# atomicarchitects/equiformer

Hardware: AMD Instinct MI355X
Metric: molecules/sec (train step) QM9 L_max=2, 6 blocks (higher is better)
Workload: dtype f32; 1 GPU; QM9 graph_attention_transformer_nonlinear_l2 train step (radius graph + fwd + L1 + bwd + AdamW), 128 molecules/GPU x 18 atoms, r=5.0, num_basis=128, alpha_drop=0.2; global_batch=128, nodes_per_gpu=2304, edges_per_gpu=25354, parallelism=dp1, matrix_mode=split, hip_graph=True, hip_graph_replays=455, hip_graph_eager_steps=3

## Files before the change

### equiformer_amd/csrc/common.h

```cpp
#pragma once
#include <hip/hip_runtime.h>
#include <stdint.h>
#include "../../include/equiformer_hip.h"

#define EQF_CHECK_LAUNCH()                      \
  do {                                          \
    hipError_t e__ = hipGetLastError();         \
    if (e__ != hipSuccess) return (int)e__;     \
  } while (0)

static inline int eqf_cdiv(long a, long b) { return (int)((a + b - 1) / b); }

__device__ __forceinline__ float wave_sum(float v) {
#pragma unroll
  for (int o = 32; o > 0; o >>= 1) v += __shfl_xor(v, o);
  return v;
}
__device__ __forceinline__ float wave_max(float v) {
#pragma unroll
  for (int o = 32; o > 0; o >>= 1) v = fmaxf(v, __shfl_xor(v, o));
  return v;
}
__device__ __forceinline__ float half_sum(float v) {
#pragma unroll
  for (int o = 16; o > 0; o >>= 1) v += __shfl_xor(v, o);
  return v;
}

__device__ __forceinline__ float sigmoidf_(float x) { return 1.0f / (1.0f + __expf(-x)); }

__device__ __forceinline__ long row_off2(int i, int d, int ld, int inner) {
  if (d == 1) return (long)i * ld;
  int q;
  if (i < (1 << 21)) q = (int)(((float)i + 0.5f) * __builtin_amdgcn_rcpf((float)d));
  else q = i / d;
  int r = i - q * d;
  return (long)q * ld + (long)r * inner;
}

struct SmallDiv {
  int d;
  float inv;
  __device__ __forceinline__ explicit SmallDiv(int d_) : d(d_), inv(1.0f / (float)d_) {}
  __device__ __forceinline__ int div(int t) const { return (int)(((float)t + 0.5f) * inv); }
};

__host__ __device__ inline int irreps_dim(const eqf_irreps& ir) {
  int D = 0;
  for (int s = 0; s < ir.nseg; ++s) D += ir.mul[s] * (2 * ir.l[s] + 1);
  return D;
}
```

### equiformer_amd/csrc/gemmx.hip

```cpp
#include <climits>
#include "sfcx_common.h"

namespace {

constexpr int GX_BK = 32;
constexpr int GX_LDK = 40;
constexpr int GX_T = 64;
constexpr int GX_ROW = GX_T * GX_LDK;
constexpr int GX_MAXP = 24;

typedef __bf16 bf16x4_t __attribute__((ext_vector_type(4)));

struct GRows {
  const float* base;
  int d, ld, inner;
};

struct GXP {
  GRows A, B, C;
  const float* bias;
  float* cs;
  float* Cw;
  int ldc;
  int M, N, K;
  int accumulate, kind;
  int vecA, vecB;
  int steps_per_split;
};
static_assert(sizeof(GXP) * GX_MAXP + 4 * (2 * GX_MAXP + 3) <= 4000, "kernarg segment");
struct GXGroup {
  int n;
  int woff[GX_MAXP + 1];
  GXP p[GX_MAXP];
};

__device__ __forceinline__ int flat_problem(const GXGroup& g, int b) {
  int pi = 0;
#pragma unroll
  for (int j = 1; j < GX_MAXP; ++j) pi += (int)((unsigned)(g.woff[j] - 1 - b) >> 31);
  return pi;
}

template <int NP>
__device__ __forceinline__ void split_n(const float* v, int n, __bf16 (*p)[8]) {
#pragma unroll
  for (int j = 0; j < 8; ++j) {
    if (j >= n) break;
    float r = v[j];
#pragma unroll
    for (int q = 0; q < NP; ++q) {
      const __bf16 h = (__bf16)r;
      p[q][j] = h;
      if (q + 1 < NP) r = r - (float)h;
    }
  }
}

template <int NP>
struct LoaderKC {
  float4 v[2];
  long roff[2];
  bool rv[2];
  __device__ __forceinline__ void init(const GRows& R, int x0, int X) {
    const int xr0 = threadIdx.x >> 3;
#pragma unroll
    for (int pass = 0; pass < 2; ++pass) {
      const int x = x0 + xr0 + 32 * pass;
      rv[pass] = x < X;
      roff[pass] = row_off2(rv[pass] ? x : x0, R.d, R.ld, R.inner);
    }
  }
  int krem;
  template <bool VEC>
  __device__ __forceinline__ void issue(const GRows& R, int k0, int K) {
    const int k = k0 + 4 * (threadIdx.x & 7);
    krem = K - k;
    if constexpr (VEC) {
      const int kc = krem > 0 ? k : 0;
#pragma unroll
      for (int pass = 0; pass < 2; ++pass) v[pass] = *reinterpret_cast<const float4*>(R.base + roff[pass] + kc);
    } else {
#pragma unroll
      for (int pass = 0; pass < 2; ++pass) {
        const float* const p = R.base + roff[pass];
        v[pass] = make_float4(p[min(k, K - 1)], p[min(k + 1, K - 1)], p[min(k + 2, K - 1)], p[min(k + 3, K - 1)]);
      }
    }
  }
  __device__ __forceinline__ void commit(__bf16* __restrict__ T) const {
    const int kq = threadIdx.x & 7, xr0 = threadIdx.x >> 3;
#pragma unroll
    for (int pass = 0; pass < 2; ++pass) {
      float f[4] = {v[pass].x, v[pass].y, v[pass].z, v[pass].w};
#pragma unroll
      for (int e = 0; e < 4; ++e)
        if (!(rv[pass] && e < krem)) f[e] = 0.f;
      __bf16 p[NP][8];
      split_n<NP>(f, 4, p);
#pragma unroll
      for (int q = 0; q < NP; ++q)
        *reinterpret_cast<bf16x4_t*>(T + q * GX_ROW + (xr0 + 32 * pass) * GX_LDK + 4 * kq) =
            bf16x4_t{p[q][0], p[q][1], p[q][2], p[q][3]};
    }
  }
};

template <int NP>
struct LoaderKS {
  float v[8];
// ... 70 lines not shown
  for (int half = 0; half < 2; ++half) {
    __builtin_amdgcn_fence(__ATOMIC_ACQ_REL, "wavefront");
    __builtin_amdgcn_wave_barrier();
#pragma unroll
    for (int q8 = 0; q8 < 8; ++q8) T[((q8 & 3) + 8 * (q8 >> 2) + 4 * hi) * GX_ST_LD + r] = acc[8 * half + q8];
    __builtin_amdgcn_fence(__ATOMIC_ACQ_REL, "wavefront");
    __builtin_amdgcn_wave_barrier();
#pragma unroll
    for (int k = 0; k < 2; ++k) {
      const int lr = rr + 8 * k, grow = row0 + 16 * half + lr;
      f32x4 v = *reinterpret_cast<const f32x4*>(T + lr * GX_ST_LD + c4);
      if (grow < M && col0 + c4 < N) {
        float* const p = rowptr(grow) + (col0 + c4);
        if (accumulate) {
          const f32x4 o = *reinterpret_cast<const f32x4*>(p);
          v[0] += o[0], v[1] += o[1], v[2] += o[2], v[3] += o[3];
        }
        *reinterpret_cast<f32x4*>(p) = v;
      }
    }
  }
}

template <int MODE, int BKIND, bool VEC>
__global__ __launch_bounds__(256) void gemmx_rows_kernel(const GXGroup g_byval) {
  KERNARG_IN_PLACE(GXGroup);
  constexpr int NA = Planes<MODE>::A, NB = Planes<MODE>::W;
  const int pi = flat_problem(g, (int)blockIdx.x);
  const GXP& P = g.p[pi];
  const int local = (int)blockIdx.x - g.woff[pi], tiles_n = (P.N + GX_T - 1) / GX_T;
  const int mt = local / tiles_n;
  const int m0 = mt * GX_T, n0 = (local - mt * tiles_n) * GX_T;
  __shared__ __attribute__((aligned(16))) __bf16 As[2][NA * GX_ROW];
  __shared__ __attribute__((aligned(16))) __bf16 Bs[2][NB * GX_ROW];
  const int wave = threadIdx.x >> 6;
  const int wm0 = (wave >> 1) * 32, wn0 = (wave & 1) * 32;
  f32x16 acc;
#pragma unroll
  for (int q = 0; q < 16; ++q) acc[q] = 0.f;

  LoaderKC<NA> la;
  LoaderKC<NB> lbk;
  LoaderKS<NB> lbs;
  la.init(P.A, m0, P.M);
  la.template issue<VEC>(P.A, 0, P.K);
  if constexpr (BKIND == 1) {
    lbk.init(P.B, n0, P.N);
    lbk.template issue<VEC>(P.B, 0, P.K);
  } else {
    lbs.init(P.B, 0);
    lbs.issue(P.B, P.K, n0, P.N);
  }
  la.commit(As[0]);
  if constexpr (BKIND == 1) lbk.commit(Bs[0]);
  else lbs.commit(Bs[0], false);
  __syncthreads();
  int cur = 0;
  for (int k0 = 0; k0 < P.K; k0 += GX_BK) {
    const bool more = k0 + GX_BK < P.K;
    if (more) {
      la.template issue<VEC>(P.A, k0 + GX_BK, P.K);
      if constexpr (BKIND == 1) lbk.template issue<VEC>(P.B, k0 + GX_BK, P.K);
      else lbs.issue(P.B, P.K, n0, P.N);
    }
    gx_mma<NA, NB>(As[cur], Bs[cur], wm0, wn0, acc);
    if (more) {
      la.commit(As[cur ^ 1]);
      if constexpr (BKIND == 1) lbk.commit(Bs[cur ^ 1]);
      else lbs.commit(Bs[cur ^ 1], false);
    }
    __syncthreads();
    cur ^= 1;
  }

  const int lane = threadIdx.x & 63, r = lane & 31, hi = lane >> 5;
  const int col = n0 + wn0 + r;
  const float bv = (P.bias && col < P.N) ? P.bias[col] : 0.f;
  const bool flat_c = P.C.d == 1;
  const SmallDiv cdiv(P.C.d);
  float* const cbase = const_cast<float*>(P.C.base);
  const int rb = m0 + wm0 + 4 * hi;
  static_assert(sizeof(As) >= 4 * GX_ST_FLOATS * sizeof(float), "the operand stages double as the store tiles");
  if (((P.C.ld | P.C.inner | P.N) & 3) == 0 && (reinterpret_cast<size_t>(cbase) & 15) == 0) {
#pragma unroll
    for (int q = 0; q < 16; ++q) acc[q] += bv;
    gx_store_tile16(acc, reinterpret_cast<float*>(&As[0][0]) + wave * GX_ST_FLOATS, m0 + wm0, P.M, n0 + wn0, P.N, P.accumulate != 0,
                    lane, [&](const int grow) {
                      if (flat_c) return cbase + (long)grow * P.C.ld;
                      const int qd = grow / P.C.d;
// ... 29 lines not shown
    }
  }
}

constexpr int GW_K = 64;
constexpr int GW_LDK = GW_K + 8;
constexpr int GW_ROW = GX_T * GW_LDK;

template <int NP>
struct LoaderWide {
  float4 v[GW_K / 16];
  int kv;
  __device__ __forceinline__ void issue(const GRows& R, int x0, int X, int K, bool two_level) {
    const int row = x0 + (threadIdx.x >> 2), q = threadIdx.x & 3;
    const bool rv = row < X;
    kv = rv ? K : 0;
    const long off = two_level ? row_off2(rv ? row : x0, R.d, R.ld, R.inner) : (long)(rv ? row : x0) * R.ld;
#pragma unroll
    for (int j = 0; j < GW_K / 16; ++j) {
      const int k = 4 * (q + 4 * j);
      v[j] = *reinterpret_cast<const float4*>(R.base + off + (k < K ? k : 0));
    }
  }
  __device__ __forceinline__ void commit(__bf16* __restrict__ T) const {
    const int row = threadIdx.x >> 2, q = threadIdx.x & 3;
#pragma unroll
    for (int j = 0; j < GW_K / 16; ++j) {
      const bool ok = 4 * (q + 4 * j) < kv;
      const float f[4] = {ok ? v[j].x : 0.f, ok ? v[j].y : 0.f, ok ? v[j].z : 0.f, ok ? v[j].w : 0.f};
      __bf16 p[NP][8];
      split_n<NP>(f, 4, p);
#pragma unroll
      for (int pl = 0; pl < NP; ++pl)
        *reinterpret_cast<bf16x4_t*>(T + pl * GW_ROW + row * GW_LDK + 4 * (q + 4 * j)) = bf16x4_t{p[pl][0], p[pl][1], p[pl][2], p[pl][3]};
    }
  }
};

template <int MODE>
__global__ __launch_bounds__(256) void gemmx_rows_wide_kernel(const GXGroup g_byval) {
  KERNARG_IN_PLACE(GXGroup);
  constexpr int NA = Planes<MODE>::A, NB = Planes<MODE>::W;
  const GXP& P = g.p[blockIdx.z];
  const int m0 = blockIdx.x * GX_T;
  if (m0 >= P.M) return;
  __shared__ __attribute__((aligned(16))) __bf16 As[NA * GW_ROW];
  __shared__ __attribute__((aligned(16))) __bf16 Bs[NB * GW_ROW];
  __shared__ __attribute__((aligned(16))) float St[4 * GX_ST_FLOATS];
  const int wave = threadIdx.x >> 6, lane = threadIdx.x & 63, r = lane & 31, hi = lane >> 5;
  const int wm0 = (wave >> 1) * 32, wn0 = (wave & 1) * 32;
  LoaderWide<NA> la;
  LoaderWide<NB> lb;
  la.issue(P.A, m0, P.M, P.K, true);
  lb.issue(P.B, 0, P.N, P.K, false);
  la.commit(As);
  const bool flat_c = P.C.d == 1;
  const SmallDiv cdiv(P.C.d);
  float* const cbase = const_cast<float*>(P.C.base);
  const int rb = m0 + wm0 + 4 * hi;
  long off0;
  int rem0 = 0;
  if (flat_c) {
    off0 = (long)rb * P.C.ld;
  } else {
    const int qb = rb / P.C.d;
    rem0 = rb - qb * P.C.d;
    off0 = (long)qb * P.C.ld;
  }
  const int nkt = (P.K + 15) / 16;
  const bool vec_c = ((P.C.ld | P.C.inner | P.N) & 3) == 0 && (reinterpret_cast<size_t>(cbase) & 15) == 0;
  for (int n0 = 0; n0 < P.N; n0 += GX_T) {
    __syncthreads();
    lb.commit(Bs);
    __syncthreads();
    if (n0 + GX_T < P.N) lb.issue(P.B, n0 + GX_T, P.N, P.K, false);
    f32x16 acc;
#pragma unroll
// ... 89 lines not shown
    __syncthreads();
    cur ^= 1;
  }
  {
    const int x = threadIdx.x & 63;
    if (csA && m0 + x < P.M) atomicAdd(P.cs + m0 + x, la.cs);
    if (csB && n0 + x < P.N) atomicAdd(P.cs + n0 + x, lb.cs);
  }
  const int lane = threadIdx.x & 63, r = lane & 31, hi = lane >> 5;
  const int col = n0 + wn0 + r;
  if (col >= P.N) return;
#pragma unroll
  for (int q = 0; q < 16; ++q) {
    const int row = m0 + wm0 + (q & 3) + 8 * (q >> 2) + 4 * hi;
    if (row < P.M) atomicAdd(P.Cw + (long)row * P.ldc + col, acc[q]);
  }
}

inline bool aligned16(const void* p) { return (reinterpret_cast<uintptr_t>(p) & 15) == 0; }
inline bool rows_vec_ok(const float* base, const eqf_rows& r) { return aligned16(base) && (r.ld % 4 == 0) && (r.inner % 4 == 0); }

static int g_gemmx_tn_minsteps = 8;

}

extern "C" {

int eqf_gemmx_group(const eqf_gemm_desc* d, int n, int mode, void* stream) {
  if (!d || n < 1 || n > GX_MAXP || mode < 0 || mode > 2) return EQF_E_BADARG;
  hipStream_t st = (hipStream_t)stream;
  for (int i = 0; i < n; ++i) {
    if (d[i].kind < 0 || d[i].kind > 3) return EQF_E_BADARG;
    if (!d[i].A || !d[i].B || !d[i].C || d[i].ra.d < 1 || d[i].rc.d < 1) return EQF_E_BADARG;
    if (d[i].kind < 2 && d[i].K < 1) return EQF_E_BADARG;
  }
  static thread_local GXGroup G;
  for (int kind = 0; kind < 2; ++kind) {
    memset(&G, 0, sizeof G);
    int maxm = 0, big = 0, wide_ok = 1, vec_ok = 1, wg = 0;
    double flops = 0, bytes = 0;
    for (int i = 0; i < n; ++i) {
      if (d[i].kind != kind || d[i].M <= 0 || d[i].N <= 0) continue;
      GXP& P = G.p[G.n];
      G.woff[G.n++] = wg;
      wg += eqf_cdiv(d[i].M, GX_T) * eqf_cdiv(d[i].N, GX_T);
      P.A = {d[i].A, d[i].ra.d, d[i].ra.ld, d[i].ra.inner};
      P.B = {d[i].B, 1, d[i].ldb, 0};
      P.C = {d[i].C, d[i].rc.d, d[i].rc.ld, d[i].rc.inner};
      P.bias = d[i].bias;
      P.M = d[i].M, P.N = d[i].N, P.K = d[i].K, P.accumulate = d[i].accumulate, P.kind = kind;
      P.vecA = rows_vec_ok(d[i].A, d[i].ra);
      P.vecB = aligned16(d[i].B) && d[i].ldb % 4 == 0;
      if (P.K % 4 != 0 || !P.vecA || (kind == 1 && !P.vecB)) vec_ok = 0;
      if (!(kind == 1 && P.K <= GW_K && P.K % 4 == 0 && P.vecA && P.vecB && P.M >= 8192 && P.N >= 2 * GX_T)) wide_ok = 0;
      if (eqf_cdiv(P.M, GX_T) > maxm) maxm = eqf_cdiv(P.M, GX_T);
      if (P.M >= 32768 / 2 + 1) big = 1;
      flops += 2.0 * P.M * (double)P.N * P.K;
      bytes += 4.0 * ((double)P.M * P.K + (double)P.K * P.N + (double)P.M * P.N);
    }
    if (G.n == 0) continue;
    const bool wide = kind == 1 && wide_ok;
    for (int i = G.n; i <= GX_MAXP; ++i) G.woff[i] = i == G.n ? wg : INT_MAX;
    const dim3 grid = wide ? dim3(maxm, 1, G.n) : dim3(wg, 1, 1);
    const int pid = eqf_prof_begin(kind == 0 ? (big ? "gemmx_group_kn_edge" : "gemmx_group_kn_node")
                                             : (big ? "gemmx_group_nk_edge" : "gemmx_group_nk_node"), st, flops, bytes);
#define GX_ROWS(M_)                                                                                              \
  do {                                                                                                           \
    if (wide) {                                                                                                  \
      hipLaunchKernelGGL((gemmx_rows_wide_kernel<M_>), grid, dim3(256), 0, st, G);                              \
    } else if (kind == 0) {                                                                                      \
      if (vec_ok) hipLaunchKernelGGL((gemmx_rows_kernel<M_, 0, true>), grid, dim3(256), 0, st, G);              \
      else hipLaunchKernelGGL((gemmx_rows_kernel<M_, 0, false>), grid, dim3(256), 0, st, G);                    \
    } else {                                                                                                     \
      if (vec_ok) hipLaunchKernelGGL((gemmx_rows_kernel<M_, 1, true>), grid, dim3(256), 0, st, G);              \
      else hipLaunchKernelGGL((gemmx_rows_kernel<M_, 1, false>), grid, dim3(256), 0, st, G);                    \
    }                                                                                                            \
  } while (0)
    if (mode == 0) GX_ROWS(0);
    else if (mode == 1) GX_ROWS(1);
    else GX_ROWS(2);
#undef GX_ROWS
    eqf_prof_end(pid, st);
    EQF_CHECK_LAUNCH();
  }
  {
    memset(&G, 0, sizeof G);
    int big = 0, wg = 0;
    double flops = 0, bytes = 0;
    for (int i = 0; i < n; ++i) {
      if (d[i].kind != 2 && d[i].kind != 3) continue;
      if (d[i].M <= 0 || d[i].N <= 0 || d[i].K <= 0) continue;
// ... 12 lines not shown
      ksplit = eqf_cdiv(total_steps, P.steps_per_split);
      G.woff[G.n] = wg;
      wg += tiles * ksplit;
      G.n++;
      if (P.K >= 32768 / 2 + 1) big = 1;
      flops += 2.0 * P.M * (double)P.N * P.K;
      bytes += 4.0 * ((double)P.K * P.M + (double)P.K * P.N + (double)P.M * P.N);
    }
    if (G.n > 0) {
      for (int i = G.n; i <= GX_MAXP; ++i) G.woff[i] = i == G.n ? wg : INT_MAX;
      const dim3 grid(wg, 1, 1);
      const int pid = eqf_prof_begin(big ? "gemmx_group_tn_edge" : "gemmx_group_tn_node", st, flops, bytes);
      if (mode == 0) hipLaunchKernelGGL((gemmx_tn_kernel<0>), grid, dim3(256), 0, st, G);
      else if (mode == 1) hipLaunchKernelGGL((gemmx_tn_kernel<1>), grid, dim3(256), 0, st, G);
      else hipLaunchKernelGGL((gemmx_tn_kernel<2>), grid, dim3(256), 0, st, G);
      eqf_prof_end(pid, st);
      EQF_CHECK_LAUNCH();
    }
  }
  return 0;
}

}
```

### equiformer_amd/csrc/rowops.hip

```cpp
#include "common.h"

namespace {

constexpr int WAVES_PER_BLOCK = 4;

struct SegTab {
  int nseg;
  int off[EQF_MAX_SEG];
  int len[EQF_MAX_SEG];
  int mul[EQF_MAX_SEG];
  int l[EQF_MAX_SEG];
  int woff[EQF_MAX_SEG];
  int boff[EQF_MAX_SEG];
  int zidx[EQF_MAX_SEG];
  int n0;
  int D;
};

SegTab make_segtab(const eqf_irreps& ir) {
  SegTab t{};
  t.nseg = ir.nseg;
  int off = 0, w = 0, b = 0, n0 = 0;
  for (int s = 0; s < ir.nseg; ++s) {
    t.off[s] = off;
// ... 307 lines not shown
    o.x = c * g.x * dsilu(v.x), o.y = c * g.y * dsilu(v.y), o.z = c * g.z * dsilu(v.z), o.w = c * g.w * dsilu(v.w);
    reinterpret_cast<float4*>(dx)[i] = o;
  }
  if (i == 0)
    for (long j = n4 * 4; j < n; ++j) dx[j] = c * dy[j] * dsilu(x[j]);
}

__global__ __launch_bounds__(256) void lnsilu_fwd_kernel(const float* __restrict__ x, const float* __restrict__ gamma,
                                                         const float* __restrict__ beta, float* __restrict__ y, int rows,
                                                         int C, float eps, int G) {
  const long ld = (long)G * C;
  {
    const int g_ = blockIdx.y * C;
    x += g_;
    gamma += g_;
    beta += g_;
    y += g_;
  }
  const int lane = threadIdx.x & 63;
  const int row = blockIdx.x * WAVES_PER_BLOCK + (threadIdx.x >> 6);
  if (row >= rows) return;
  const bool act = lane < C;
  const float v = act ? x[(long)row * ld + lane] : 0.f;
  const float mean = wave_sum(v) / C;
  const float d = act ? v - mean : 0.f;
  const float rs = rsqrtf(wave_sum(d * d) / C + eps);
  if (act) {
    const float z = d * rs * gamma[lane] + beta[lane];
    y[(long)row * ld + lane] = z * sigmoidf_(z);
  }
}

__global__ __launch_bounds__(256) void lnsilu_bwd_kernel(const float* __restrict__ x, const float* __restrict__ gamma,
                                                         const float* __restrict__ beta, const float* __restrict__ dy,
                                                         float* __restrict__ dx, float* __restrict__ d_gamma,
                                                         float* __restrict__ d_beta, int rows, int C, float eps, int G) {
  const long ld = (long)G * C;
  {
    const int g_ = blockIdx.y * C;
    x += g_;
    gamma += g_;
    beta += g_;
    dy += g_;
    dx += g_;
    d_gamma += g_;
    d_beta += g_;
  }
  const int lane = threadIdx.x & 63;
  const int wave_global = blockIdx.x * WAVES_PER_BLOCK + (threadIdx.x >> 6);
  const int nwaves = gridDim.x * WAVES_PER_BLOCK;
  const bool act = lane < C;
  const float gm = act ? gamma[lane] : 0.f, bt = act ? beta[lane] : 0.f;
  float acc_g = 0.f, acc_b = 0.f;
// ... 410 lines not shown
```

### equiformer_amd/lib.py

```python
import ctypes
import os

_HERE = os.path.dirname(os.path.abspath(__file__))
LIB_PATH = os.path.join(_HERE, "libequiformer_hip.so")
if os.environ.get("EQF_LIB_VARIANT"):
    LIB_PATH = os.path.join(_HERE, "libequiformer_hip_%s.so" % os.environ["EQF_LIB_VARIANT"])

EQF_MAX_SEG = 8
EQF_MAX_PATHS = 72

c_fp = ctypes.c_void_p
c_int = ctypes.c_int


class EqfIrreps(ctypes.Structure):
    _fields_ = [("nseg", c_int), ("l", c_int * EQF_MAX_SEG), ("mul", c_int * EQF_MAX_SEG), ("odd", c_int * EQF_MAX_SEG)]


class EqfRows(ctypes.Structure):
    _fields_ = [("d", c_int), ("ld", c_int), ("inner", c_int)]


class EqfGemmDesc(ctypes.Structure):
    _fields_ = [("A", c_fp), ("B", c_fp), ("C", c_fp), ("bias", c_fp), ("ra", EqfRows), ("rc", EqfRows),
# ... 27 lines not shown
    "eqf_radius_graph_pbc_fill": [c_fp, c_fp, c_fp, c_int, _f, c_int, c_fp, c_fp, c_fp, c_fp, c_fp, c_fp, c_fp, c_fp],
    "eqf_sumsq": [c_fp, ctypes.c_long, c_fp, c_fp],
    "eqf_adamw_step": [c_fp, c_fp, c_fp, c_fp, c_fp, c_fp, c_fp, ctypes.c_long, _f, _f, _f, _f, c_int, _f, _f, c_fp],
    "eqf_adamw_step_dev": [c_fp, c_fp, c_fp, c_fp, c_fp, c_fp, c_fp, ctypes.c_long, c_fp, _f, _f, _f, _f, _f, c_fp],
    "eqf_segment_ptr": [c_fp, c_int, c_int, c_fp, c_fp, c_fp],
    "eqf_exclusive_scan_i32": [c_fp, c_int, c_fp, c_fp, c_fp],
    "eqf_csr_by_source": [c_fp, c_fp, c_fp, c_int, c_int, c_fp, c_fp, c_fp],
    "eqf_csr_by_source_multi": [c_fp, c_fp, c_fp, c_int, c_int, c_fp, c_fp, c_fp],
    "eqf_graph_pad_tail": [c_int, c_int, c_int, c_int, c_int, c_fp, c_fp, c_fp, c_fp, c_fp, c_fp, c_fp, c_fp, c_fp, c_fp],
    "eqf_edge_geom_fwd": [c_fp, c_fp, c_fp, c_fp, c_int, c_int, c_fp, c_fp, c_fp, c_fp],
    "eqf_edge_geom_bwd": [c_fp, c_fp, c_fp, c_int, c_int, c_fp, c_fp],
    "eqf_rbf_gaussian_fwd": [c_fp, c_int, c_int, c_fp, c_fp, c_fp, c_fp, _f, c_fp, c_fp],
    "eqf_rbf_gaussian_bwd": [c_fp, c_fp, c_int, c_int, c_fp, c_fp, c_fp, c_fp, _f, c_fp, c_fp, c_fp, c_fp, c_fp, c_fp],
    "eqf_rbf_expnorm_fwd": [c_fp, c_int, c_int, c_fp, c_fp, _f, _f, c_fp, c_fp],
    "eqf_rbf_expnorm_bwd": [c_fp, c_fp, c_int, c_int, c_fp, c_fp, _f, _f, c_fp, c_fp],
    "eqf_rbf_bessel_fwd": [c_fp, c_int, c_int, c_fp, _f, c_fp, c_fp],
    "eqf_rbf_bessel_bwd": [c_fp, c_fp, c_int, c_int, c_fp, _f, c_fp, c_fp, c_fp],
    "eqf_gemm_nn": [c_fp, EqfRows, c_fp, c_int, c_fp, EqfRows, c_fp, c_int, c_int, c_int, c_int, c_fp],
    "eqf_gemm_nt": [c_fp, EqfRows, c_fp, c_int, c_fp, EqfRows, c_fp, c_int, c_int, c_int, c_int, c_fp],
    "eqf_gemm_tn": [c_fp, EqfRows, c_fp, EqfRows, c_fp, c_int, c_int, c_int, c_int, c_fp],
    "eqf_gemm_tn_colsum": [c_fp, EqfRows, c_fp, EqfRows, c_fp, c_int, c_int, c_int, c_int, c_fp, c_fp, c_fp],
    "eqf_gemm_group": [ctypes.POINTER(EqfGemmDesc), c_int, c_fp],
    "eqf_gemmx_group": [ctypes.POINTER(EqfGemmDesc), c_int, c_int, c_fp],
    "eqf_colsum": [c_fp, EqfRows, c_int, c_int, c_fp, c_fp],
    "eqf_dtp_coupling_fwd": [c_fp, c_fp, _P_PATHS, c_fp, c_int, c_fp],
    "eqf_dtp_coupling_bwd": [c_fp, c_fp, _P_PATHS, c_fp, c_int, c_fp],
    "eqf_dtp_linear_fwd": [c_fp, c_fp, c_fp, _P_PATHS, _PP, c_fp, c_fp, _P_IRR, c_int, c_fp],
    "eqf_dtp_linear_wgrad": [c_fp, c_fp, c_fp, _P_PATHS, c_fp, _P_IRR, _PP, c_int, c_fp],
    "eqf_sfc_fwd": [c_fp, c_fp, c_fp, _P_PATHS, _PP, c_fp, c_fp, c_fp, c_fp, _P_IRR, c_fp, c_int, c_int, c_fp],
    "eqf_sfc_bwd_data": [c_fp, c_fp, c_fp, _P_PATHS, _PP, c_fp, c_fp, _P_IRR, c_fp, c_int, c_fp, c_fp, c_fp, c_int, c_fp],
    "eqf_sfc_bwd_weight": [c_fp, c_fp, c_fp, _P_PATHS, c_fp, _P_IRR, c_fp, c_int, _PP, c_fp, c_int, c_fp],
    "eqf_sfcx_packed_numel": [_P_PATHS, _P_IRR, c_int, c_int],
    "eqf_sfcx_supported": [_P_PATHS, _P_IRR, c_int, c_int],
    "eqf_sfcx_fwd_gated": [c_fp, ctypes.POINTER(EqfGateIn), c_fp, c_fp, _P_PATHS, c_fp, c_fp, c_fp, _P_IRR, c_int, c_int, c_fp],
    "eqf_sfcx_bwd_data_gated": [c_fp, ctypes.POINTER(EqfGateIn), c_fp, c_fp, _P_PATHS, c_fp, c_fp, _P_IRR, c_fp, c_fp, c_fp,
                                c_int, c_int, c_fp],
    "eqf_sfcx_bwd_weight_gated": [c_fp, ctypes.POINTER(EqfGateIn), c_fp, c_fp, _P_PATHS, c_fp, _P_IRR, _PP, c_int, c_int,
                                  c_fp],
    "eqf_sfcx_bwd_weight_bias": [c_fp, c_fp, c_fp, _P_PATHS, c_fp, _P_IRR, c_fp, c_int, _PP, c_fp, c_fp, c_fp, c_int, c_int, c_fp],
    "eqf_sfcx_bwd_weight_gated_bias": [c_fp, ctypes.POINTER(EqfGateIn), c_fp, c_fp, _P_PATHS, c_fp, _P_IRR, _PP, c_fp, c_int,
                                       c_int, c_fp],
    "eqf_sfcx_pack": [_PP, c_fp, _P_PATHS, _P_IRR, c_int, c_int, c_fp, c_fp],
    "eqf_sfcx_fwd": [c_fp, c_fp, c_fp, _P_PATHS, c_fp, c_fp, c_fp, c_fp, _P_IRR, c_fp, c_int, c_int, c_int, c_fp],
    "eqf_sfcx_bwd_data": [c_fp, c_fp, c_fp, _P_PATHS, c_fp, c_fp, _P_IRR, c_fp, c_int, c_fp, c_fp, c_fp, c_int, c_int, c_fp],
    "eqf_sfcx_bwd_weight": [c_fp, c_fp, c_fp, _P_PATHS, c_fp, _P_IRR, c_fp, c_int, _PP, c_fp, c_int, c_int, c_fp],
    "eqf_layernorm_fwd": [c_fp, c_fp, c_fp, c_fp, c_fp, c_fp, c_int, _P_IRR, _f, c_fp],
# ... 143 lines not shown
```

### equiformer_amd/nets/graph_attention_transformer.py

```python
import torch
from torch import nn

from .. import ops
from ..graph import EdgeGraph
from ..irreps import Irreps
from .layers import (Activation, EdgeContext, EdgeDegreeEmbeddingNetwork, EquivariantLayerNormV2,
                     FeedForwardNetwork, FullyConnectedTensorProductRescale, GaussianRadialBasisLayer, GraphAttention,
                     LinearRS, NodeEmbeddingNetwork, RadialBank, RadialBasis, ScaledScatter, SeparableFCTP, TransBlock, get_norm_layer)
from .registry import register_model

_RESCALE = True
_USE_BIAS = True

_MAX_ATOM_TYPE = 5
_AVG_NUM_NODES = 18.03065905448718
_AVG_DEGREE = 15.57930850982666


class _Trunk(nn.Module):

    def _build_trunk(self, irreps_node_embedding, num_layers, irreps_node_attr, irreps_sh, max_radius,
                     number_of_basis, fc_neurons, irreps_feature, irreps_head, num_heads, irreps_pre_attn,
                     rescale_degree, nonlinear_message, irreps_mlp_mid, norm_layer, alpha_drop, proj_drop, out_drop,
                     drop_path_rate, max_atom_type, avg_degree, avg_num_nodes):
# ... 65 lines not shown
        no_wd_list = []
        named = {name for name, _ in self.named_parameters()}
        for module_name, module in self.named_modules():
            if isinstance(module, (nn.Linear, nn.LayerNorm, EquivariantLayerNormV2, GaussianRadialBasisLayer, RadialBasis)):
                for parameter_name, _ in module.named_parameters():
                    if isinstance(module, nn.Linear) and "weight" in parameter_name:
                        continue
                    full = module_name + "." + parameter_name
                    assert full in named
                    no_wd_list.append(full)
        return set(no_wd_list)

    def set_fused(self, flag):
        for m in self.modules():
            if hasattr(m, "use_fused"):
                m.use_fused = "legacy" if flag == "legacy" else bool(flag)

    def _radial_bank(self):
        bank = self.__dict__.get("_bank")
        if bank is None:
            mods = [self.edge_deg_embed.rad]
            for attn in [blk.attention for blk in self.blocks] + self._attention_heads():
                mods.append(attn.radial_module())
            bank = RadialBank(mods)
            self.__dict__["_bank"] = bank
        return bank if (bank.ok and self.use_radial_bank) else None

    use_radial_bank = True
    _block_cls = TransBlock

    def late_gradient_parameters(self):
        bank = self._radial_bank()
        return [p for m in bank.modules for p in m.parameters()] if bank is not None else []

    def _attention_heads(self):
        return []

    def _trunk_forward(self, node_embedding, pos, graph, offsets=None):
        node_features, ectx = self._trunk_features(node_embedding, pos, graph, offsets)
        if isinstance(self.head, GraphAttention):
            outputs = self.head(node_features, ectx=ectx)
        else:
            outputs = self.head(node_features)
        return self.scale_scatter(outputs, graph.mol_ptr, graph.batch, graph.num_graphs)

    def _trunk_features(self, node_embedding, pos, graph, offsets=None, extra=None):
        _, edge_length, edge_sh = ops.edge_geometry(pos, offsets, graph, self.lmax_sh)
        edge_scalars = self.rbf(edge_length)
        bank = self._radial_bank()
        ectx = EdgeContext(graph, edge_sh, edge_scalars, radial_bank=bank)
        a, b = node_embedding, self.edge_deg_embed(node_embedding, ectx)
# ... 94 lines not shown
```

### equiformer_amd/nets/graph_attention_transformer_md17.py

```python
import torch

from .. import ops
from ..graph import EdgeGraph
from ..irreps import Irreps
from .graph_attention_transformer import _Trunk
from .layers import ExpNormalSmearing, GaussianRadialBasisLayer, GraphAttention, RadialBasis
from .registry import register_model

_MAX_ATOM_TYPE = 64
_AVG_NUM_NODES = 18.03065905448718
_AVG_DEGREE = 15.57930850982666


class GraphAttentionTransformerMD17(_Trunk):
    def __init__(self, irreps_in="64x0e", irreps_node_embedding="128x0e+64x1e+32x2e", num_layers=6,
                 irreps_node_attr="1x0e", irreps_sh="1x0e+1x1e+1x2e", max_radius=5.0, number_of_basis=128,
                 basis_type="gaussian", fc_neurons=[64, 64], irreps_feature="512x0e",
                 irreps_head="32x0e+16x1o+8x2e", num_heads=4, irreps_pre_attn=None, rescale_degree=False,
                 nonlinear_message=False, irreps_mlp_mid="128x0e+64x1e+32x2e", use_attn_head=False,
                 norm_layer="layer", alpha_drop=0.2, proj_drop=0.0, out_drop=0.0, drop_path_rate=0.0, mean=None,
                 std=None, scale=None, atomref=None):
        super().__init__()
        self.use_attn_head = use_attn_head
        self.task_mean, self.task_std, self.scale = mean, std, scale
        self.register_buffer("atomref", atomref)
        self.irreps_node_input = Irreps(irreps_in)
        self.basis_type = basis_type
        self._build_trunk(irreps_node_embedding, num_layers, irreps_node_attr, irreps_sh, max_radius,
                          number_of_basis, fc_neurons, irreps_feature, irreps_head, num_heads, irreps_pre_attn,
                          rescale_degree, nonlinear_message, irreps_mlp_mid, norm_layer, alpha_drop, proj_drop,
                          out_drop, drop_path_rate, _MAX_ATOM_TYPE, _AVG_DEGREE, _AVG_NUM_NODES)
        if use_attn_head:
            self.head = GraphAttention(self.irreps_feature, self.irreps_node_attr, self.irreps_edge_attr,
                                       Irreps("1x0e"), self.fc_neurons, self.irreps_head, num_heads, irreps_pre_attn,
                                       rescale_degree, nonlinear_message, alpha_drop, proj_drop)
            self.apply(self._init_weights)

    def _attention_heads(self):
        return [self.head] if self.use_attn_head else []

    def _make_rbf(self):
        if self.basis_type == "gaussian":
            self.rbf = GaussianRadialBasisLayer(self.number_of_basis, cutoff=self.max_radius)
        elif self.basis_type == "exp":
            self.rbf = ExpNormalSmearing(cutoff_lower=0.0, cutoff_upper=self.max_radius, num_rbf=self.number_of_basis,
                                         trainable=False)
        elif self.basis_type == "bessel":
            self.rbf = RadialBasis(self.number_of_basis, cutoff=self.max_radius, rbf={"name": "spherical_bessel"})
        else:
            raise ValueError

    differentiable_forces_in_eval = False

    @torch.enable_grad()
    def forward(self, node_atom, pos, batch, graph=None):
        pos = pos.to(torch.float32).contiguous().requires_grad_(True)
        if graph is None:
            graph = EdgeGraph.from_radius(pos, batch, self.max_radius, max_num_neighbors=1000)
        atom_embedding, _, _ = self.atom_embed(node_atom)
# ... 99 lines not shown
```

### equiformer_amd/nets/layers.py

```python
import math
import os

import torch
from torch import nn

from .. import ops, so3
from ..irreps import Irrep, Irreps
from ..layout import DtpTable, RowLayout

_RESCALE = True
_USE_BIAS = True


def _simplified_sorted(irreps):
    irreps = Irreps(irreps)
    s, _ = irreps.sort_even_first()
    return s.simplify()


class _TensorProductWeights(nn.Module):

    def __init__(self, weight_numel, internal):
        super().__init__()
        self.weight_numel = weight_numel
# ... 165 lines not shown
            mods.append(nn.SiLU())
        self.net = nn.Sequential(*mods)
        self.offset = nn.Parameter(torch.zeros(ch_list[-1]))
        bound = 1 / math.sqrt(ch_list[-2])
        nn.init.uniform_(self.offset, -bound, bound)

    def forward(self, f_in):
        x = f_in
        mods = list(self.net)
        i = 0
        while i < len(mods):
            lin = mods[i]
            if i == len(mods) - 1:
                return ops.dense_linear(x, lin.weight, self.offset)
            ln = mods[i + 1]
            x = ops.dense_linear(x, lin.weight, lin.bias)
            x = ops.ln_silu(x, ln.weight, ln.bias, ln.eps)
            i += 3
        return x


class RadialBank:

    def __init__(self, modules):
        self.modules = [m for m in modules if m is not None]
        mods = [list(m.net) for m in self.modules]
        self.ok = len(self.modules) >= 2 and all(
            len(ms) == 7 and ms[0].weight.shape == mods[0][0].weight.shape and ms[3].weight.shape == mods[0][3].weight.shape
            and ms[3].weight.shape[0] == ms[3].weight.shape[1] and ms[0].weight.shape[0] <= 64 for ms in mods)

    LAST_BANKED = os.environ.get("EQF_RADIAL_LAST_BANKED", "1") == "1"

    def forward(self, edge_scalars):
        ms = self.modules
        G = len(ms)
        C = ms[0].net[0].weight.shape[0]
        cat = torch.cat
        h = ops.dense_linear(edge_scalars, cat([m.net[0].weight for m in ms]), cat([m.net[0].bias for m in ms]))
        h = ops.ln_silu(h, cat([m.net[1].weight for m in ms]), cat([m.net[1].bias for m in ms]), ms[0].net[1].eps, groups=G)
        h = ops.grouped_linear(h, C, [m.net[3].weight for m in ms], [m.net[3].bias for m in ms], wide=True)
        h = ops.ln_silu(h, cat([m.net[4].weight for m in ms]), cat([m.net[4].bias for m in ms]), ms[0].net[4].eps, groups=G)
        if self.LAST_BANKED:
            outs = ops.grouped_linear(h, C, [m.net[6].weight for m in ms], [m.offset for m in ms], wide=False)
            return {id(m): o for m, o in zip(ms, outs)}
        return {id(m): hg for m, hg in zip(ms, ops.split_columns(h, G))}

    @staticmethod
    def last_layer(module, hidden):
        return ops.dense_linear(hidden, module.net[6].weight, module.offset)


class GaussianRadialBasisLayer(nn.Module):
    def __init__(self, num_basis, cutoff):
        super().__init__()
        self.num_basis, self.cutoff = num_basis, cutoff + 0.0
        self.mean = nn.Parameter(torch.zeros(1, num_basis))
        self.std = nn.Parameter(torch.zeros(1, num_basis))
        self.weight = nn.Parameter(torch.ones(1, 1))
        self.bias = nn.Parameter(torch.zeros(1, 1))
        nn.init.uniform_(self.mean, 0, 1.0)
        nn.init.uniform_(self.std, 1.0 / num_basis, 1.0)
# ... 511 lines not shown
```

### equiformer_amd/ops.py

```python
import contextlib
import ctypes
import os
import weakref

import torch
from torch.autograd import Function
from torch.autograd.function import once_differentiable

from . import lib
from .lib import EqfGemmDesc, EqfRows, call


class HipOnlyError(RuntimeError):
    pass


_dummy = {}


class _Flag:
    on = False


_input_grads_only = _Flag()
# ... 1092 lines not shown
        G, K, wide, Ns, has_b = ctx.meta
        rows_n, ldx = x.shape
        dev = x.device
        if torch.is_grad_enabled():
            dlist = [dys[0]] if wide else [(d if d is not None else _zeros((rows_n, Ns[g]), dev)) for g, d in enumerate(dys)]
            dx = _GroupedDgrad.apply(K, wide, G, *dlist, *Ws) if ctx.needs_input_grad[0] else None
            if not _want_param_grads():
                return (dx, None, None) + (None,) * (2 * G)
            outs = _GroupedWgrad.apply(K, wide, tuple(Ns), tuple(has_b), x, *dlist)
            it = iter(outs[G:])
            return (dx, None, None) + tuple(outs[:G]) + tuple((next(it) if hb else None) for hb in has_b)
        dyt, offs, ldd = _glin_views(dys, wide, Ns, rows_n, dev)
        dx = None
        if ctx.needs_input_grad[0]:
            dx = _glin_dgrad(dyt, offs, ldd, list(Ws), K, rows_n)
        if not _want_param_grads():
            return (dx, None, None) + (None,) * (2 * G)
        dWs, dbs = _glin_wgrad(dyt, offs, ldd, x, K, Ns, has_b)
        return (dx, None, None) + tuple(dWs) + tuple(dbs)


def grouped_linear(x, K, weights, biases, wide):
    return _GroupedLinear.apply(x, int(K), bool(wide), *weights, *biases)


class _FoldWeight(Function):

    @staticmethod
    def forward(ctx, W, w, row_start, w_of_row):
        W, w = _c(W), _c(w)
        _chk(W, w, row_start, w_of_row)
        out = torch.empty_like(W)
        call("eqf_fold_weight_fwd", _p(W), _p(w), _p(row_start), _p(w_of_row), _p(out), w_of_row.numel(), _stream())
        ctx.save_for_backward(W, w, row_start, w_of_row)
        return out

    @staticmethod
    def backward(ctx, g):
        W, w, row_start, w_of_row = ctx.saved_tensors
        if torch.is_grad_enabled():
            dW = _FoldWeight.apply(g, w, row_start, w_of_row)
            row_of = torch.repeat_interleave(torch.arange(w_of_row.numel(), device=W.device),
                                             (row_start[1:] - row_start[:-1]).long())
            dw = torch.zeros_like(w).index_add(0, w_of_row.long()[row_of], g * W)
            return dW, dw, None, None
        g = _c(g)
# ... 1372 lines not shown
```

### include/equiformer_hip.h

```cpp
#ifndef EQUIFORMER_HIP_H
#define EQUIFORMER_HIP_H

#ifdef __cplusplus
extern "C" {
#endif

#define EQF_MAX_SEG 8
#define EQF_MAX_PATHS 72

#define EQF_E_BADARG (-1)
#define EQF_E_UNSUPPORTED (-2)

typedef struct eqf_irreps {
  int nseg;
  int l[EQF_MAX_SEG];
  int mul[EQF_MAX_SEG];
  int odd[EQF_MAX_SEG];
} eqf_irreps;

typedef struct eqf_dtp_paths {
  int npaths;
  int sh_dim;
  int in_dim;
  int out_dim;
// ... 59 lines not shown
  int ld;
  int inner;
} eqf_rows;

int eqf_gemm_nn(const float* A, eqf_rows ra, const float* B, int ldb, float* C, eqf_rows rc,
                const float* bias, int M, int N, int K, int accumulate, void* stream);
int eqf_gemm_nt(const float* A, eqf_rows ra, const float* B, int ldb, float* C, eqf_rows rc,
                const float* bias, int M, int N, int K, int accumulate, void* stream);
int eqf_gemm_tn(const float* A, eqf_rows ra, const float* B, eqf_rows rb, float* C, int ldc, int M,
                int N, int R, void* stream);
int eqf_gemm_tn_colsum(const float* A, eqf_rows ra, const float* B, eqf_rows rb, float* C, int ldc, int M, int N,
                       int R, float* colsum_a, float* colsum_b, void* stream);

typedef struct eqf_gemm_desc {
  const float* A;
  const float* B;
  float* C;
  const float* bias;
  eqf_rows ra, rc;
  int ldb, M, N, K, accumulate, kind;
} eqf_gemm_desc;
int eqf_gemm_group(const eqf_gemm_desc* d, int n, void* stream);
int eqf_gemmx_group(const eqf_gemm_desc* d, int n, int mode, void* stream);

int eqf_colsum(const float* X, eqf_rows rx, int R, int N, float* out, void* stream);

int eqf_dtp_coupling_fwd(const float* sh, const float* cg, const eqf_dtp_paths* paths, float* coupling,
                         int E, void* stream);
int eqf_dtp_coupling_bwd(const float* d_coupling, const float* cg, const eqf_dtp_paths* paths,
                         float* d_sh, int E, void* stream);

int eqf_dtp_linear_fwd(const float* x, const float* coupling, const float* w,
                       const eqf_dtp_paths* paths, const float* const* Wl, const float* bias0,
                       float* out, const eqf_irreps* out_irreps, int E, void* stream);
int eqf_dtp_linear_wgrad(const float* x, const float* coupling, const float* w,
                         const eqf_dtp_paths* paths, const float* d_out,
                         const eqf_irreps* out_irreps, float* const* dWl, int E, void* stream);

int eqf_sfc_fwd(const float* x, const float* coupling, const float* w, const eqf_dtp_paths* paths,
                const float* const* Wl, const float* bias0, const float* W2, const float* bias2, float* out1,
                const eqf_irreps* out1_irreps, float* out2, int n2, int E, void* stream);
int eqf_sfc_bwd_data(const float* x, const float* coupling, const float* w, const eqf_dtp_paths* paths,
                     const float* const* Wl, const float* W2, const float* d_out1, const eqf_irreps* out1_irreps,
                     const float* d_out2, int n2, float* dx, float* dw, float* d_coupling, int E, void* stream);
int eqf_sfc_bwd_weight(const float* x, const float* coupling, const float* w, const eqf_dtp_paths* paths,
                       const float* d_out1, const eqf_irreps* out1_irreps, const float* d_out2, int n2,
// ... 169 lines not shown
```

Before: 14550 molecules/s.

## Fuse LayerNorm+SiLU into grouped radial GEMM A-operand loading

Adds a LN+SiLU prologue to the gemmx grouped row kernels. Per-row statistics are computed in shared memory, and the normalized, activated A tiles are applied in registers before the bf16 split. The normalized activation is still written out once, by the n0==0 tiles, so backward can use it. The radial bank uses this fused path for both LN+SiLU+linear stages, which removes separate ln_silu kernel launches and an extra read of the hidden activations. In exchange, every N-tile recomputes the row stats, and the fused path has no create_graph backward, so MD17 keeps the unfused path.

Result: no change. 14560 molecules/s (median of 2 runs) (+0.0%).

```diff
diff --git a/equiformer_amd/csrc/common.h b/equiformer_amd/csrc/common.h
--- a/equiformer_amd/csrc/common.h
+++ b/equiformer_amd/csrc/common.h
@@ -29,6 +29,20 @@
 
 __device__ __forceinline__ float sigmoidf_(float x) { return 1.0f / (1.0f + __expf(-x)); }
 
+__device__ __forceinline__ void ln_row_stats(float v, bool act, int C, float eps, float& mean, float& rs) {
+  mean = wave_sum(v) / C;
+  const float d = act ? v - mean : 0.f;
+  float q = __builtin_fmaf(d, d, __shfl_xor(d * d, 32));
+#pragma unroll
+  for (int o = 16; o > 0; o >>= 1) q += __shfl_xor(q, o);
+  rs = rsqrtf(q / C + eps);
+}
+__device__ __forceinline__ float lnsilu_apply(float v, float mean, float rs, float gm, float bt) {
+  const float d = v - mean;
+  const float z = __builtin_fmaf(d * rs, gm, bt);
+  return z * sigmoidf_(z);
+}
+
 __device__ __forceinline__ long row_off2(int i, int d, int ld, int inner) {
   if (d == 1) return (long)i * ld;
   int q;
diff --git a/equiformer_amd/csrc/gemmx.hip b/equiformer_amd/csrc/gemmx.hip
--- a/equiformer_amd/csrc/gemmx.hip
+++ b/equiformer_amd/csrc/gemmx.hip
@@ -7,6 +7,7 @@
 constexpr int GX_LDK = 40;
 constexpr int GX_T = 64;
 constexpr int GX_ROW = GX_T * GX_LDK;
+constexpr int GX_LN_C = 64;
 constexpr int GX_MAXP = 24;
 
 typedef __bf16 bf16x4_t __attribute__((ext_vector_type(4)));
@@ -21,17 +22,21 @@
   const float* bias;
   float* cs;
   float* Cw;
+  float* ln_y;
   int ldc;
   int M, N, K;
   int accumulate, kind;
   int vecA, vecB;
   int steps_per_split;
+  int ln_off;
 };
 static_assert(sizeof(GXP) * GX_MAXP + 4 * (2 * GX_MAXP + 3) <= 4000, "kernarg segment");
 struct GXGroup {
   int n;
   int woff[GX_MAXP + 1];
   GXP p[GX_MAXP];
+  const float *ln_g, *ln_b;
+  float ln_eps;
 };
 
 __device__ __forceinline__ int flat_problem(const GXGroup& g, int b) {
@@ -54,6 +59,27 @@
       if (q + 1 < NP) r = r - (float)h;
     }
   }
+}
+
+__device__ __forceinline__ void gx_ln_stats(const GRows& R, int x0, int X, float eps, float* __restrict__ mean_s,
+                                            float* __restrict__ rs_s) {
+  const int wave = threadIdx.x >> 6, lane = threadIdx.x & 63;
+  float v[16];
+#pragma unroll
+  for (int i = 0; i < 16; ++i) {
+    const int x = x0 + 16 * wave + i;
+    v[i] = R.base[(long)(x < X ? x : x0) * R.ld + lane];
+  }
+#pragma unroll
+  for (int i = 0; i < 16; ++i) {
+    float mean, rs;
+    ln_row_stats(v[i], true, GX_LN_C, eps, mean, rs);
+    if (lane == 0) mean_s[16 * wave + i] = mean, rs_s[16 * wave + i] = rs;
+  }
+}
+__device__ __forceinline__ float4 gx_lnsilu4(const float4 v, float mean, float rs, const float4 g, const float4 b) {
+  return make_float4(lnsilu_apply(v.x, mean, rs, g.x, b.x), lnsilu_apply(v.y, mean, rs, g.y, b.y),
+                     lnsilu_apply(v.z, mean, rs, g.z, b.z), lnsilu_apply(v.w, mean, rs, g.w, b.w));
 }
 
 template <int NP>
@@ -85,6 +111,16 @@
         const float* const p = R.base + roff[pass];
         v[pass] = make_float4(p[min(k, K - 1)], p[min(k + 1, K - 1)], p[min(k + 2, K - 1)], p[min(k + 3, K - 1)]);
       }
+    }
+  }
+  __device__ __forceinline__ void lnsilu(const GRows& R, int k0, const float* __restrict__ mean_s, const float* __restrict__ rs_s,
+                                         const float* __restrict__ gm, const float* __restrict__ bt, float* __restrict__ y) {
+    const int k = k0 + 4 * (threadIdx.x & 7), xr0 = threadIdx.x >> 3;
+    const float4 g4 = *reinterpret_cast<const float4*>(gm + k), b4 = *reinterpret_cast<const float4*>(bt + k);
+#pragma unroll
+    for (int pass = 0; pass < 2; ++pass) {
+      v[pass] = gx_lnsilu4(v[pass], mean_s[xr0 + 32 * pass], rs_s[xr0 + 32 * pass], g4, b4);
+      if (y && rv[pass]) *reinterpret_cast<float4*>(y + roff[pass] + k) = v[pass];
     }
   }
   __device__ __forceinline__ void commit(__bf16* __restrict__ T) const {
@@ -201,7 +237,7 @@
   }
 }
 
-template <int MODE, int BKIND, bool VEC>
+template <int MODE, int BKIND, bool VEC, bool LN = false>
 __global__ __launch_bounds__(256) void gemmx_rows_kernel(const GXGroup g_byval) {
   KERNARG_IN_PLACE(GXGroup);
   constexpr int NA = Planes<MODE>::A, NB = Planes<MODE>::W;
@@ -230,6 +266,15 @@
     lbs.init(P.B, 0);
     lbs.issue(P.B, P.K, n0, P.N);
   }
+  __shared__ float ln_mean[LN ? GX_T : 1], ln_rs[LN ? GX_T : 1];
+  const float* const ln_g = LN ? g.ln_g + P.ln_off : nullptr;
+  const float* const ln_b = LN ? g.ln_b + P.ln_off : nullptr;
+  float* const ln_y = LN && n0 == 0 ? P.ln_y : nullptr;
+  if constexpr (LN) {
+    gx_ln_stats(P.A, m0, P.M, g.ln_eps, ln_mean, ln_rs);
+    __syncthreads();
+    la.lnsilu(P.A, 0, ln_mean, ln_rs, ln_g, ln_b, ln_y);
+  }
   la.commit(As[0]);
   if constexpr (BKIND == 1) lbk.commit(Bs[0]);
   else lbs.commit(Bs[0], false);
@@ -244,6 +289,7 @@
     }
     gx_mma<NA, NB>(As[cur], Bs[cur], wm0, wn0, acc);
     if (more) {
+      if constexpr (LN) la.lnsilu(P.A, k0 + GX_BK, ln_mean, ln_rs, ln_g, ln_b, ln_y);
       la.commit(As[cur ^ 1]);
       if constexpr (BKIND == 1) lbk.commit(Bs[cur ^ 1]);
       else lbs.commit(Bs[cur ^ 1], false);
@@ -319,6 +365,17 @@
       v[j] = *reinterpret_cast<const float4*>(R.base + off + (k < K ? k : 0));
     }
   }
+  __device__ __forceinline__ void lnsilu(const GRows& R, int x0, const float* __restrict__ mean_s, const float* __restrict__ rs_s,
+                                         const float* __restrict__ gm, const float* __restrict__ bt, float* __restrict__ y) {
+    const int row = threadIdx.x >> 2, q = threadIdx.x & 3;
+    const float mean = mean_s[row], rs = rs_s[row];
+#pragma unroll
+    for (int j = 0; j < GW_K / 16; ++j) {
+      const int k = 4 * (q + 4 * j);
+      v[j] = gx_lnsilu4(v[j], mean, rs, *reinterpret_cast<const float4*>(gm + k), *reinterpret_cast<const float4*>(bt + k));
+      if (kv > 0) *reinterpret_cast<float4*>(y + (long)(x0 + row) * R.ld + k) = v[j];
+    }
+  }
   __device__ __forceinline__ void commit(__bf16* __restrict__ T) const {
     const int row = threadIdx.x >> 2, q = threadIdx.x & 3;
 #pragma unroll
@@ -334,7 +391,7 @@
   }
 };
 
-template <int MODE>
+template <int MODE, bool LN = false>
 __global__ __launch_bounds__(256) void gemmx_rows_wide_kernel(const GXGroup g_byval) {
   KERNARG_IN_PLACE(GXGroup);
   constexpr int NA = Planes<MODE>::A, NB = Planes<MODE>::W;
@@ -350,6 +407,12 @@
   LoaderWide<NB> lb;
   la.issue(P.A, m0, P.M, P.K, true);
   lb.issue(P.B, 0, P.N, P.K, false);
+  if constexpr (LN) {
+    __shared__ float ln_mean[GX_T], ln_rs[GX_T];
+    gx_ln_stats(P.A, m0, P.M, g.ln_eps, ln_mean, ln_rs);
+    __syncthreads();
+    la.lnsilu(P.A, m0, ln_mean, ln_rs, g.ln_g + P.ln_off, g.ln_b + P.ln_off, P.ln_y);
+  }
   la.commit(As);
   const bool flat_c = P.C.d == 1;
   const SmallDiv cdiv(P.C.d);
@@ -485,11 +548,26 @@
 
 static int g_gemmx_tn_minsteps = 8;
 
-}
-
-extern "C" {
-
-int eqf_gemmx_group(const eqf_gemm_desc* d, int n, int mode, void* stream) {
+struct GXLn {
+  const float *x, *gamma, *beta;
+  float eps;
+  float* y;
+};
+
+int plan_lnsilu(const eqf_gemm_desc* d, int n, const GXLn& ln) {
+  if (!ln.x || !ln.gamma || !ln.beta || !ln.y) return EQF_E_BADARG;
+  if (n < 2) return EQF_E_UNSUPPORTED;
+  if (!aligned16(ln.x) || !aligned16(ln.y) || !aligned16(ln.gamma) || !aligned16(ln.beta)) return EQF_E_UNSUPPORTED;
+  for (int i = 0; i < n; ++i) {
+    if (d[i].kind != 1 || d[i].K != GX_LN_C || d[i].ra.d != 1 || d[i].ra.ld != d[0].ra.ld || d[i].accumulate) return EQF_E_UNSUPPORTED;
+    if (!rows_vec_ok(d[i].A, d[i].ra) || !aligned16(d[i].B) || d[i].ldb % 4 != 0) return EQF_E_UNSUPPORTED;
+    const long off = d[i].A - ln.x;
+    if (off < 0 || off + GX_LN_C > d[i].ra.ld) return EQF_E_UNSUPPORTED;
+  }
+  return 0;
+}
+
+int gemmx_group(const eqf_gemm_desc* d, int n, int mode, const GXLn* ln, void* stream) {
   if (!d || n < 1 || n > GX_MAXP || mode < 0 || mode > 2) return EQF_E_BADARG;
   hipStream_t st = (hipStream_t)stream;
   for (int i = 0; i < n; ++i) {
@@ -497,9 +575,14 @@
     if (!d[i].A || !d[i].B || !d[i].C || d[i].ra.d < 1 || d[i].rc.d < 1) return EQF_E_BADARG;
     if (d[i].kind < 2 && d[i].K < 1) return EQF_E_BADARG;
   }
+  if (ln) {
+    const int rc = plan_lnsilu(d, n, *ln);
+    if (rc) return rc;
+  }
   static thread_local GXGroup G;
   for (int kind = 0; kind < 2; ++kind) {
     memset(&G, 0, sizeof G);
+    if (ln) G.ln_g = ln->gamma, G.ln_b = ln->beta, G.ln_eps = ln->eps;
     int maxm = 0, big = 0, wide_ok = 1, vec_ok = 1, wg = 0;
     double flops = 0, bytes = 0;
     for (int i = 0; i < n; ++i) {
@@ -514,6 +597,7 @@
       P.M = d[i].M, P.N = d[i].N, P.K = d[i].K, P.accumulate = d[i].accumulate, P.kind = kind;
       P.vecA = rows_vec_ok(d[i].A, d[i].ra);
       P.vecB = aligned16(d[i].B) && d[i].ldb % 4 == 0;
+      if (ln) P.ln_off = GX_LN_C * i, P.ln_y = ln->y + (d[i].A - ln->x);
       if (P.K % 4 != 0 || !P.vecA || (kind == 1 && !P.vecB)) vec_ok = 0;
       if (!(kind == 1 && P.K <= GW_K && P.K % 4 == 0 && P.vecA && P.vecB && P.M >= 8192 && P.N >= 2 * GX_T)) wide_ok = 0;
       if (eqf_cdiv(P.M, GX_T) > maxm) maxm = eqf_cdiv(P.M, GX_T);
@@ -529,7 +613,10 @@
                                              : (big ? "gemmx_group_nk_edge" : "gemmx_group_nk_node"), st, flops, bytes);
 #define GX_ROWS(M_)                                                                                              \
   do {                                                                                                           \
-    if (wide) {                                                                                                  \
+    if (ln) {                                                                                                    \
+      if (wide) hipLaunchKernelGGL((gemmx_rows_wide_kernel<M_, true>), grid, dim3(256), 0, st, G);              \
+      else hipLaunchKernelGGL((gemmx_rows_kernel<M_, 1, true, true>), grid, dim3(256), 0, st, G);               \
+    } else if (wide) {                                                                                           \
       hipLaunchKernelGGL((gemmx_rows_wide_kernel<M_>), grid, dim3(256), 0, st, G);                              \
     } else if (kind == 0) {                                                                                      \
       if (vec_ok) hipLaunchKernelGGL((gemmx_rows_kernel<M_, 0, true>), grid, dim3(256), 0, st, G);              \
@@ -588,3 +675,15 @@
 }
 
 }
+
+extern "C" {
+
+int eqf_gemmx_group(const eqf_gemm_desc* d, int n, int mode, void* stream) { return gemmx_group(d, n, mode, nullptr, stream); }
+
+int eqf_gemmx_group_lnsilu(const eqf_gemm_desc* d, int n, int mode, const float* x, const float* gamma, const float* beta,
+                           float eps, float* y, void* stream) {
+  const GXLn ln = {x, gamma, beta, eps, y};
+  return gemmx_group(d, n, mode, &ln, stream);
+}
+
+}
diff --git a/equiformer_amd/csrc/rowops.hip b/equiformer_amd/csrc/rowops.hip
--- a/equiformer_amd/csrc/rowops.hip
+++ b/equiformer_amd/csrc/rowops.hip
@@ -353,13 +353,9 @@
   if (row >= rows) return;
   const bool act = lane < C;
   const float v = act ? x[(long)row * ld + lane] : 0.f;
-  const float mean = wave_sum(v) / C;
-  const float d = act ? v - mean : 0.f;
-  const float rs = rsqrtf(wave_sum(d * d) / C + eps);
-  if (act) {
-    const float z = d * rs * gamma[lane] + beta[lane];
-    y[(long)row * ld + lane] = z * sigmoidf_(z);
-  }
+  float mean, rs;
+  ln_row_stats(v, act, C, eps, mean, rs);
+  if (act) y[(long)row * ld + lane] = lnsilu_apply(v, mean, rs, gamma[lane], beta[lane]);
 }
 
 __global__ __launch_bounds__(256) void lnsilu_bwd_kernel(const float* __restrict__ x, const float* __restrict__ gamma,
diff --git a/equiformer_amd/lib.py b/equiformer_amd/lib.py
--- a/equiformer_amd/lib.py
+++ b/equiformer_amd/lib.py
@@ -73,6 +73,7 @@
     "eqf_gemm_tn_colsum": [c_fp, EqfRows, c_fp, EqfRows, c_fp, c_int, c_int, c_int, c_int, c_fp, c_fp, c_fp],
     "eqf_gemm_group": [ctypes.POINTER(EqfGemmDesc), c_int, c_fp],
     "eqf_gemmx_group": [ctypes.POINTER(EqfGemmDesc), c_int, c_int, c_fp],
+    "eqf_gemmx_group_lnsilu": [ctypes.POINTER(EqfGemmDesc), c_int, c_int, c_fp, c_fp, c_fp, _f, c_fp, c_fp],
     "eqf_colsum": [c_fp, EqfRows, c_int, c_int, c_fp, c_fp],
     "eqf_dtp_coupling_fwd": [c_fp, c_fp, _P_PATHS, c_fp, c_int, c_fp],
     "eqf_dtp_coupling_bwd": [c_fp, c_fp, _P_PATHS, c_fp, c_int, c_fp],
diff --git a/equiformer_amd/nets/graph_attention_transformer.py b/equiformer_amd/nets/graph_attention_transformer.py
--- a/equiformer_amd/nets/graph_attention_transformer.py
+++ b/equiformer_amd/nets/graph_attention_transformer.py
@@ -111,11 +111,12 @@
             mods = [self.edge_deg_embed.rad]
             for attn in [blk.attention for blk in self.blocks] + self._attention_heads():
                 mods.append(attn.radial_module())
-            bank = RadialBank(mods)
+            bank = RadialBank(mods, fused=self.radial_fused)
             self.__dict__["_bank"] = bank
         return bank if (bank.ok and self.use_radial_bank) else None
 
     use_radial_bank = True
+    radial_fused = True
     _block_cls = TransBlock
 
     def late_gradient_parameters(self):
diff --git a/equiformer_amd/nets/graph_attention_transformer_md17.py b/equiformer_amd/nets/graph_attention_transformer_md17.py
--- a/equiformer_amd/nets/graph_attention_transformer_md17.py
+++ b/equiformer_amd/nets/graph_attention_transformer_md17.py
@@ -35,6 +35,8 @@
                                        Irreps("1x0e"), self.fc_neurons, self.irreps_head, num_heads, irreps_pre_attn,
                                        rescale_degree, nonlinear_message, alpha_drop, proj_drop)
             self.apply(self._init_weights)
+
+    radial_fused = False
 
     def _attention_heads(self):
         return [self.head] if self.use_attn_head else []
diff --git a/equiformer_amd/nets/layers.py b/equiformer_amd/nets/layers.py
--- a/equiformer_amd/nets/layers.py
+++ b/equiformer_amd/nets/layers.py
@@ -211,7 +211,8 @@
 
 class RadialBank:
 
-    def __init__(self, modules):
+    def __init__(self, modules, fused=True):
+        self.fused = fused
         self.modules = [m for m in modules if m is not None]
         mods = [list(m.net) for m in self.modules]
         self.ok = len(self.modules) >= 2 and all(
@@ -226,6 +227,15 @@
         C = ms[0].net[0].weight.shape[0]
         cat = torch.cat
         h = ops.dense_linear(edge_scalars, cat([m.net[0].weight for m in ms]), cat([m.net[0].bias for m in ms]))
+        if self.fused:
+            h = ops.ln_silu_grouped_linear(h, cat([m.net[1].weight for m in ms]), cat([m.net[1].bias for m in ms]),
+                                           ms[0].net[1].eps, C, [m.net[3].weight for m in ms], [m.net[3].bias for m in ms], wide=True)
+            g2, b2 = cat([m.net[4].weight for m in ms]), cat([m.net[4].bias for m in ms])
+            if self.LAST_BANKED:
+                outs = ops.ln_silu_grouped_linear(h, g2, b2, ms[0].net[4].eps, C, [m.net[6].weight for m in ms],
+                                                  [m.offset for m in ms], wide=False)
+                return {id(m): o for m, o in zip(ms, outs)}
+            return {id(m): hg for m, hg in zip(ms, ops.split_columns(ops.ln_silu(h, g2, b2, ms[0].net[4].eps, groups=G), G))}
         h = ops.ln_silu(h, cat([m.net[1].weight for m in ms]), cat([m.net[1].bias for m in ms]), ms[0].net[1].eps, groups=G)
         h = ops.grouped_linear(h, C, [m.net[3].weight for m in ms], [m.net[3].bias for m in ms], wide=True)
         h = ops.ln_silu(h, cat([m.net[4].weight for m in ms]), cat([m.net[4].bias for m in ms]), ms[0].net[4].eps, groups=G)
diff --git a/equiformer_amd/ops.py b/equiformer_amd/ops.py
--- a/equiformer_amd/ops.py
+++ b/equiformer_amd/ops.py
@@ -1138,6 +1138,70 @@
 
 def grouped_linear(x, K, weights, biases, wide):
     return _GroupedLinear.apply(x, int(K), bool(wide), *weights, *biases)
+
+
+_EQF_E_UNSUPPORTED = -2
+
+
+def _lnsilu_glin_fwd(x, gamma, beta, eps, K, wide, Ws, bs):
+    G = len(Ws)
+    rows_n, ldx = x.shape
+    m = _MATRIX_MODES[_matrix_mode[0]] if _gemmx[0] else None
+    h = torch.empty_like(x)
+    if m is not None and G <= 24 and rows_n > 0:
+        Ns = [int(W.shape[0]) for W in Ws]
+        if wide:
+            out = torch.empty((rows_n, sum(Ns)), device=x.device, dtype=torch.float32)
+            outs, ldo, offs = [out] * G, sum(Ns), [sum(Ns[:g]) for g in range(G)]
+        else:
+            outs = [torch.empty((rows_n, n), device=x.device, dtype=torch.float32) for n in Ns]
+            ldo, offs = None, [0] * G
+        descs = [_desc(1, (x, g * K), rows(1, ldx, 0), (Ws[g], 0), K, (outs[g], offs[g]),
+                       rows(1, ldo if wide else Ns[g], 0), bs[g], rows_n, Ns[g], K) for g in range(G)]
+        rc = lib.load().eqf_gemmx_group_lnsilu((EqfGemmDesc * G)(*descs), G, m, _p(x), _p(gamma), _p(beta), eps, _p(h), _stream())
+        if rc == 0:
+            return h, (out if wide else tuple(outs)), True
+        if rc != _EQF_E_UNSUPPORTED:
+            raise lib.HipLibraryError("eqf_gemmx_group_lnsilu failed with code %d" % rc)
+    call("eqf_lnsilu_group_fwd", _p(x), _p(gamma), _p(beta), _p(h), rows_n, ldx // G, G, eps, _stream())
+    return h, _glin_fwd(h, K, wide, Ws, bs), False
+
+
+class _LnSiluGroupedLinear(Function):
+
+    last_fused = None
+
+    @staticmethod
+    def forward(ctx, x, gamma, beta, eps, K, wide, *params):
+        G = len(params) // 2
+        Ws, bs = params[:G], params[G:]
+        x = _c(x)
+        _chk(x, gamma, beta, *Ws, *bs)
+        assert x.shape[1] == G * K and all(W.shape[1] == K and W.is_contiguous() for W in Ws)
+        h, out, _LnSiluGroupedLinear.last_fused = _lnsilu_glin_fwd(x, gamma, beta, eps, K, wide, list(Ws), list(bs))
+        ctx.save_for_backward(x, gamma, beta, h, *Ws)
+        ctx.meta = (G, K, wide, [int(W.shape[0]) for W in Ws], [b is not None for b in bs], eps)
+        return out
+
+    @staticmethod
+    def backward(ctx, *dys):
+        if torch.is_grad_enabled():
+            raise HipOnlyError("the fused LN+SiLU grouped linear has no create_graph backward: build the RadialBank with "
+                               "fused=False")
+        x, gamma, beta, h, *Ws = ctx.saved_tensors
+        G, K, wide, Ns, has_b, eps = ctx.meta
+        rows_n = x.shape[0]
+        dyt, offs, ldd = _glin_views(dys, wide, Ns, rows_n, x.device)
+        dh = _glin_dgrad(dyt, offs, ldd, list(Ws), K, rows_n)
+        dWs, dbs = _glin_wgrad(dyt, offs, ldd, h, K, Ns, has_b)
+        dx = torch.empty_like(x)
+        dg, db = _zeros2(gamma.numel(), beta.numel(), x.device)
+        call("eqf_lnsilu_group_bwd", _p(x), _p(gamma), _p(beta), _p(dh), _p(dx), _p(dg), _p(db), rows_n, K, G, eps, _stream())
+        return (dx, dg, db, None, None, None) + tuple(dWs) + tuple(dbs)
+
+
+def ln_silu_grouped_linear(x, gamma, beta, eps, K, weights, biases, wide):
+    return _LnSiluGroupedLinear.apply(x, gamma, beta, float(eps), int(K), bool(wide), *weights, *biases)
 
 
 class _FoldWeight(Function):
diff --git a/include/equiformer_hip.h b/include/equiformer_hip.h
--- a/include/equiformer_hip.h
+++ b/include/equiformer_hip.h
@@ -105,6 +105,8 @@
 } eqf_gemm_desc;
 int eqf_gemm_group(const eqf_gemm_desc* d, int n, void* stream);
 int eqf_gemmx_group(const eqf_gemm_desc* d, int n, int mode, void* stream);
+int eqf_gemmx_group_lnsilu(const eqf_gemm_desc* d, int n, int mode, const float* x, const float* gamma, const float* beta,
+                           float eps, float* y, void* stream);
 
 int eqf_colsum(const float* X, eqf_rows rx, int R, int N, float* out, void* stream);
 
```
